# jiaxi98/cnf_ot

Hardware: AMD Instinct MI355X
Metric: MC samples/sec through flow fwd+log|detJ| at dim=2, batch=65536 (higher is better)
Workload: dtype f32; 1 GPU; configs[1]: OT free dim=2, batch=65536, sample_and_log_prob (RQS fwd + log|detJ|), L=2 H=16 M=2 K=5, params N(0,0.20^2) seed 42; ONE STEP = one evaluator-shaped pass of 10000 time-slices x 65536 samples (cnf_ot/utils.py:311-340), each slice its own condition t, one cnf_sample_logprob call per rank; batch=65536, dim=2, parallelism=slice-shard x1 (contiguous blocks of the step's slices; no collective)

## Files before the change

cnf_ot_amd/csrc/cnf_flow.hip:

```cpp
#include "cnf_common.h"
#include <cstdlib>
#include "cnf_pwl_build.h"

#include <math.h>
#include <new>
#include <stdlib.h>
#include <string.h>

namespace cnf {


enum CMode { C_SINGLE = 0, C_PER_SAMPLE = 1, C_TILE_UNIFORM = 2, C_GENERIC = 3 };
enum AuxMode { AUX_LOGDET = 0, AUX_LOGPROB = 1 };


template <class R> struct FlowArgsT {
  ModelArgs m;
  const R* in;
  const R* c;
  R* out;
  R* aux;
  int64_t B;
  int64_t c_block;
  int32_t c_mode, aux_mode;
// ... 296 lines not shown
    T o, ld, olo;
    const bool last = step == a.L - 1;
    [[maybe_unused]] R* clo = nullptr;
    if constexpr (PRECISE) {
      clo = LO + SPL * threadIdx.x;
      const T vlo = step == 0 ? splat<T>(0.0f) : lds_get<T>(clo, first_idx, TS);
      table_spline_precise<K, FAST>(tab, tabd, lds_get<T>(cu, first_idx, TS), vlo, sc, o, ld, olo);
      lds_put(clo, first_idx, TS, olo);
      if (last) bacc->add(o, olo);
    } else {
      table_spline<K, INV, FAST, T>(tab, lds_get<T>(cu, first_idx, TS), sc, o, ld);
    }
    lds_put(co, first_idx, TS, o);
    acc += ld;
    uniform_ptr w = weights + l * a.per_layer;
    const float* wq = a.wq + l * a.per_layer_q;
    for (int d = 1; d < D; ++d) {
      const int i = first_idx + d * idx_step;
      T th[P];
      if constexpr (MFMA && !std::is_same<T, double>::value) {
        conditioner_mfma<T>(reinterpret_cast<const f4*>(wq), d, a.M, c, TO_BASE ? co : cu, first_idx, idx_step, TS, th,
                            D >= 3 ? w : nullptr);
        wq += cond_floats_mfma(d, a.M);
        w += cond_floats(d, H, a.M, P);
      } else {
        conditioner<H, P, T, PERIODIC>(w, d, a.M, c, TO_BASE ? co : cu, first_idx, idx_step, TS, th);
        w += cond_floats_p(d, H, a.M, P, PERIODIC);
      }
      if constexpr (PRECISE) {
        const T vlo = step == 0 ? splat<T>(0.0f) : lds_get<T>(clo, i, TS);
        cond_spline_precise<K, FAST, false>(th, lds_get<T>(cu, i, TS), vlo, sc, a.scd, e2tab, o, ld, olo);
        lds_put(clo, i, TS, olo);
        if (last) bacc->add(o, olo);
      } else {
        cond_spline<K, INV, FAST, T>(th, lds_get<T>(cu, i, TS), sc, o, ld);
      }
      lds_put(co, i, TS, o);
      acc += ld;
    }
    R* t = U; U = O; O = t;
  }
  return acc;
}

__device__ __forceinline__ void store_aux(float* aux, int64_t i, int64_t B, float r) {
  if (i < B) aux[i] = r;
}
__device__ __forceinline__ void store_aux(double* aux, int64_t i, int64_t B, double r) {
  if (i < B) aux[i] = r;
}
__device__ __forceinline__ void store_aux(float* aux, int64_t i, int64_t B, v2f r) {
  if (i + 1 < B && ((reinterpret_cast<uintptr_t>(aux + i) & 7) == 0)) *reinterpret_cast<v2f*>(aux + i) = r;
  else { if (i < B) aux[i] = r.x; if (i + 1 < B) aux[i + 1] = r.y; }
}

template <int H, int K, bool TO_BASE, bool FAST, class T, bool MFMA = false, bool PRECISE = false, bool PERIODIC = false, int DFIX = 0>
__global__ __launch_bounds__(TILE, 2) void flow_kernel(const FlowArgsT<typename Lanes<T>::real> a) {
  typedef typename Lanes<T>::real R;
  extern __shared__ __attribute__((aligned(16))) float lds_raw[];
  R* lds = reinterpret_cast<R*>(lds_raw);
  constexpr int HDR = hdr_floats(K);
  constexpr int SPL = Lanes<T>::N;
  constexpr int TS = TILE * SPL;
  const int DD = DFIX ? DFIX : a.m.D;
  const uint32_t dmagic = DFIX == 2 ? 0x80000000u : (uint32_t)a.div_magic;
  R* tab = lds;
  R* U = lds + HDR;
  R* O = U + DD * TS;
  if (gate_closed(a)) return;
  for (int i = threadIdx.x; i < HDR; i += TILE) tab[i] = table_of<R>(a.m)[i];
  [[maybe_unused]] double* e2tab = nullptr;
  [[maybe_unused]] double* tabd = nullptr;
  [[maybe_unused]] R* LO = nullptr;
  if constexpr (PRECISE) {
    LO = O + DD * TS;
    e2tab = reinterpret_cast<double*>(LO + DD * TS);
    tabd = e2tab + EXP2_N;
    for (int i = threadIdx.x; i < EXP2_N; i += TILE) e2tab[i] = a.m.e2tab[i];
    for (int i = threadIdx.x; i < HDR; i += TILE) tabd[i] = a.m.tabd[i];
  }

  const int64_t n_tiles = (a.B + TS - 1) / TS;
  for (int64_t tile = blockIdx.x; tile < n_tiles; tile += gridDim.x) {
    const int64_t tile_start = tile * TS;
    const int64_t i = tile_start + SPL * threadIdx.x;
    __syncthreads();
    if (TO_BASE && !PRECISE && a.fd2) tile_load_fd<R>(a, U, DD, dmagic, TS, tile_start);
    else if (a.in) tile_load<R>(a.in, U, DD, dmagic, TS, tile_start, a.B);
    else tile_noise_flow(a, U, DD, dmagic, TS, tile_start, TILE);
    const T c = load_cond<T>(a, tile_start, i);
    __syncthreads();

    T base = splat<T>(0.0f);
    if (!TO_BASE && a.aux_mode == AUX_LOGPROB && a.aux) base = base_logprob<T>(lds_col<T>(U + SPL * threadIdx.x, TS), DD);
    BaseAcc<T> bacc;
    [[maybe_unused]] T poison = splat<T>(0.0f);
    if constexpr (TO_BASE) {
      for (int d = 0; d < DD; ++d) { const T v = lds_get<T>(U + SPL * threadIdx.x, d, TS); poison += v - v; }
    }
    const T acc = flow_pass<H, K, TO_BASE, FAST, T, MFMA, PRECISE, PERIODIC, DFIX>(a.m, tab, U, O, c, e2tab, tabd, LO, &bacc);
    if (a.aux) {
      T r = acc;
      if (a.aux_mode == AUX_LOGPROB) {
        if constexpr (PRECISE) r = bacc.log_prob(acc, DD);
        else r = TO_BASE ? base_logprob<T>(lds_col<T>(U + SPL * threadIdx.x, TS), DD) + acc : base - acc;
      }
      if constexpr (TO_BASE) r += poison;
      if (TO_BASE && !PRECISE && a.fd2) store_fd(a, i, r);
      else store_aux(a.aux, i, a.B, r);
    }
    if (a.out) {
      if constexpr (TO_BASE) {
        for (int d = 0; d < DD; ++d) lds_put(U + SPL * threadIdx.x, d, TS, lds_get<T>(U + SPL * threadIdx.x, d, TS) + poison);
      }
      __syncthreads();
      tile_store<R>(a.out, U, DD, dmagic, TS, tile_start, a.B);
    }
  }
}


template <class R>
__device__ __forceinline__ void tile_load_n(const R* __restrict__ g, R* U, int D, uint32_t magic, int TS,
                                            int64_t tile_start, int64_t B, int nthreads) {
  const int64_t base = tile_start * D;
  const int n_el = (int)(B - tile_start < TS ? B - tile_start : TS) * D;
  for (int e = threadIdx.x; e < TS * D; e += nthreads) {
    const int s = magic ? (int)__umulhi((uint32_t)e, magic) : e, d = e - s * D;
    U[d * TS + s] = e < n_el ? g[base + e] : (R)0;
  }
}
template <class R>
__device__ __forceinline__ void tile_store_n(R* __restrict__ g, const R* U, int D, uint32_t magic, int TS,
                                             int64_t tile_start, int64_t B, int nthreads) {
  const int64_t base = tile_start * D;
  const int n_el = (int)(B - tile_start < TS ? B - tile_start : TS) * D;
  for (int e = threadIdx.x; e < n_el; e += nthreads) {
    const int s = magic ? (int)__umulhi((uint32_t)e, magic) : e, d = e - s * D;
    g[base + e] = U[d * TS + s];
  }
}

template <int H, int K, bool FAST, class T>
__global__ __launch_bounds__(1024) void flow_dpar_kernel(const FlowArgs a) {
  extern __shared__ __attribute__((aligned(16))) float lds[];
  constexpr int HDR = hdr_floats(K), P = 3 * K + 1, SPL = Lanes<T>::N, TS = 64 * SPL;
  const int D = a.m.D, L = a.m.L, NT = blockDim.x, NW = NT >> 6;
  const int wave = __builtin_amdgcn_readfirstlane(threadIdx.x >> 6), lane = threadIdx.x & 63;
  float* tab = lds;
  float* U = lds + HDR;
  float* O = U + D * TS;
  float* LD = O + D * TS;
  if (gate_closed(a)) return;
  for (int i = threadIdx.x; i < HDR; i += NT) tab[i] = a.m.prep[i];
  const SplineConsts& sc = a.m.sc;
  uniform_ptr weights = as_uniform(a.m.prep + HDR);
  const int64_t cpart = cond_floats(0, H, a.m.M, P) - H;

  const int64_t n_tiles = (a.B + TS - 1) / TS;
  for (int64_t tile = blockIdx.x; tile < n_tiles; tile += gridDim.x) {
    const int64_t tile_start = tile * TS;
    const int64_t i = tile_start + SPL * lane;
    __syncthreads();
    if (a.in) tile_load_n<float>(a.in, U, D, a.div_magic, TS, tile_start, a.B, NT);
    else tile_noise_flow(a, U, D, a.div_magic, TS, tile_start, NT);
    const T c = load_cond<T>(a, tile_start, i);
    __syncthreads();
    T base = splat<T>(0.0f);
    if (wave == 0 && a.aux_mode == AUX_LOGPROB && a.aux) base = base_logprob<T>(lds_col<T>(U + SPL * lane, TS), D);
    T acc = splat<T>(0.0f);
    for (int l = 0; l < L; ++l) {
      const bool odd = l & 1;
      const int first_idx = odd ? D - 1 : 0, idx_step = odd ? -1 : 1;
      const float* cu = U + SPL * lane;
      float* co = O + SPL * lane;
      T o, ld;
      if (wave == 0) {
        table_spline<K, true, FAST, T>(tab, lds_get<T>(cu, first_idx, TS), sc, o, ld);
        lds_put(co, first_idx, TS, o);
        acc += ld;
      }
      for (int d = 1 + wave; d < D; d += NW) {
        const int64_t off = l * a.m.per_layer + (int64_t)H * ((d - 1) + (int64_t)d * (d - 1) / 2) + (d - 1) * cpart;
        T th[P];
        conditioner<H, P, T>(weights + off, d, a.m.M, c, cu, first_idx, idx_step, TS, th);
        const int idx = first_idx + d * idx_step;
        cond_spline<K, true, FAST, T>(th, lds_get<T>(cu, idx, TS), sc, o, ld);
        lds_put(co, idx, TS, o);
        acc += ld;
      }
      __syncthreads();
      float* t = U; U = O; O = t;
    }
    if (a.aux) lds_put(LD + wave * TS + SPL * lane, 0, TS, acc);
    __syncthreads();
    if (a.aux && wave == 0) {
      T tot = splat<T>(0.0f);
      for (int w = 0; w < NW; ++w) tot += lds_get<T>(LD + w * TS + SPL * lane, 0, TS);
      store_aux(a.aux, i, a.B, a.aux_mode == AUX_LOGPROB ? base - tot : tot);
    }
    if (a.out) tile_store_n<float>(a.out, U, D, a.div_magic, TS, tile_start, a.B, NT);
  }
}

constexpr int PWL_MAX_THREADS = 1024;

struct PwlArgs {
  ModelArgs m;
  const float* in;
  float* out;
  float* aux;
  const float* tables;
  int64_t B, slice_len;
  int32_t n_slices, tiles_per_slice, aux_mode;
  const uint32_t* gate;
  uint32_t gate_epoch;
  int32_t gate_want;
  uint64_t seed;
  int64_t first_sample, slice_stride;
  int32_t in_shared;
};

__global__ void cond_uniform_kernel(const float* __restrict__ c, int64_t B, uint32_t* flag, uint32_t epoch) {
  const uint32_t c0 = __float_as_uint(c[0]);
  bool diff = false;
  for (int64_t i = blockIdx.x * (int64_t)blockDim.x + threadIdx.x; i < B; i += (int64_t)gridDim.x * blockDim.x)
    diff |= __float_as_uint(c[i]) != c0;
  if (__syncthreads_or(diff) && threadIdx.x == 0) *flag = epoch;
}

template <int K, bool TO_BASE, bool FAST, bool PRECISE = false, bool SHIFT_FREE_OK = false, int LROWS = PWL_LROWS, int LFIX = 0,
          bool LEAN_OK = false>
__device__ __forceinline__ v2f flow2_tables(const float* tab, const float* tbl, const float* __restrict__ gtbl,
                                            int L, const SplineConsts sc, v2f& u0, v2f& u1,
                                            const PreciseConsts* pc = nullptr, const double* e2tab = nullptr,
                                            const double* tabd = nullptr, BaseAcc<v2f>* bacc = nullptr) {
  constexpr bool INV = !TO_BASE;
  constexpr bool LEAN = LEAN_OK && INV && FAST;
  static_assert(!PRECISE || TO_BASE, "precise path: data -> base");
  v2f acc = splat<v2f>(0.0f);
  [[maybe_unused]] v2f lo0 = splat<v2f>(0.0f), lo1 = lo0;
  if (LFIX) L = LFIX;
#pragma unroll
  for (int step = 0; step < (LFIX ? LFIX : L); ++step) {
    const int l = TO_BASE ? L - 1 - step : step;
    const bool odd = l & 1;
    const v2f uf = odd ? u1 : u0, uo = odd ? u0 : u1;
    v2f of, oo, ld, olo_f, olo_o;
    bool general;
    const float* tl = tbl + l * pwl_ltbl(LROWS);
    const float* gl = gtbl + (int64_t)l * PWL_TBL;
    if constexpr (PRECISE) {
      table_spline_precise<K, FAST>(tab, tabd, uf, odd ? lo1 : lo0, sc, of, ld, olo_f);
      if (step == L - 1) bacc->add(of, olo_f);
      acc += ld;
      v2f th[PWL_P];
      pwl_eval<LROWS>(tl, gl, of, th, general);
      cond_spline_precise<K, FAST, true>(th, uo, odd ? lo0 : lo1, sc, *pc, e2tab, oo, ld, olo_o);
      if (step == L - 1) bacc->add(oo, olo_o);
      lo0 = odd ? olo_o : olo_f;
      lo1 = odd ? olo_f : olo_o;
    } else {
      PwlRows rr;
      v2f qa[K], qb[K];
      if (!TO_BASE) {
        pwl_find<LROWS>(tl, uf, rr, general);
        rr.dua = pwl_logit_pairs<LROWS>(rr.ra, gl, rr.pa, uf.x, qa);
        rr.dub = pwl_logit_pairs<LROWS>(rr.rb, gl, rr.pb, uf.y, qb);
      }
      constexpr bool LOGPROD = LEAN;
      bool tails = true;
      if constexpr (LEAN) tails = __builtin_amdgcn_ballot_w64(maybe_outside(uf, uo, sc.lo, sc.hi)) != 0;
      v2f larg = splat<v2f>(1.0f);
      if constexpr (LOGPROD) {
        table_spline<K, INV, FAST, v2f, true, LEAN>(tab, uf, sc, of, larg, tails);
      } else {
        table_spline<K, INV, FAST, v2f, false, LEAN>(tab, uf, sc, of, ld, tails);
        acc += ld;
      }
      if (TO_BASE) {
        pwl_find<LROWS>(tl, of, rr, general);
        rr.dua = pwl_logit_pairs<LROWS>(rr.ra, gl, rr.pa, of.x, qa);
        rr.dub = pwl_logit_pairs<LROWS>(rr.rb, gl, rr.pb, of.y, qb);
      }
      auto slopes = [&](int ka, int kb, v2f& ta, v2f& tb) {
        ta = pwl_slope_pair<LROWS>(rr.ra, gl, rr.pa, ka, rr.dua);
        tb = pwl_slope_pair<LROWS>(rr.rb, gl, rr.pb, kb, rr.dub);
      };
      if (!SHIFT_FREE_OK || __builtin_amdgcn_ballot_w64(general) != 0)
      {
        cond_spline_rows<K, INV, FAST, false, false, LEAN>(qa, qb, slopes, uo, sc, oo, ld, tails);
        if constexpr (LOGPROD) { const v2f lg = Math<FAST>::log(larg); ld += INV ? -lg : lg; }
      } else {
        cond_spline_rows<K, INV, FAST, true, LOGPROD, LEAN>(qa, qb, slopes, uo, sc, oo, ld, tails);
        if constexpr (LOGPROD) { const v2f lg = Math<FAST>::log(larg * ld); ld = INV ? -lg : lg; }
      }
    }
    acc += ld;
    u0 = odd ? oo : of;
    u1 = odd ? of : oo;
  }
  return acc;
}

template <int K, bool TO_BASE, bool FAST, bool PRECISE = false, int LROWS = PWL_LROWS, int LFIX = 0, bool SEEDED = false>
__global__ __launch_bounds__(PWL_MAX_THREADS) void flow_pwl_kernel(const PwlArgs a) {
  const int PWL_THREADS = blockDim.x, PWL_TS = 2 * PWL_THREADS;
  extern __shared__ __attribute__((aligned(16))) float lds_raw[];
  constexpr int HDR = (hdr_floats(K) + 3) & ~3;
  float* tab = lds_raw;
  float* tbl = lds_raw + HDR;
  const int tid = threadIdx.x;
  const int L = LFIX ? LFIX : a.m.L;
  if (gate_closed(a)) return;
  for (int i = tid; i < hdr_floats(K); i += PWL_THREADS) tab[i] = table_of<float>(a.m)[i];
  const SplineConsts sc = sc_scalars(sc_of<float>(a.m));
  [[maybe_unused]] double* e2tab = nullptr;
  [[maybe_unused]] double* tabd = nullptr;
  if constexpr (PRECISE) {
    e2tab = reinterpret_cast<double*>(tbl + L * pwl_ltbl(LROWS));
    tabd = e2tab + EXP2_N;
    for (int i = tid; i < EXP2_N; i += PWL_THREADS) e2tab[i] = a.m.e2tab[i];
    for (int i = tid; i < hdr_floats(K); i += PWL_THREADS) tabd[i] = a.m.tabd[i];
  }

  const int total = a.n_slices * a.tiles_per_slice;
  const int per_block = (total + gridDim.x - 1) / gridDim.x;
  const int t0 = blockIdx.x * per_block;
  const int t1 = t0 + per_block < total ? t0 + per_block : total;
  int cur = -1;
  struct Tile { int slice; int ti; int valid; int64_t g0; int64_t st0; int64_t gin; };
  auto tile_at = [&](int slice, int ti) {
    Tile t;
    t.slice = slice;
    t.ti = ti;
    const int64_t s0 = (int64_t)t.slice * a.slice_len;
    const int64_t len = a.B - s0 < a.slice_len ? a.B - s0 : a.slice_len;
    const int64_t jt = (int64_t)ti * PWL_TS;
    const int64_t left = len - jt;
    t.valid = left >= PWL_TS ? PWL_TS : (left > 0 ? (int)left : 0);
    t.g0 = s0 + jt;
    t.gin = a.in_shared ? jt : t.g0;
    t.st0 = a.first_sample + (int64_t)t.slice * a.slice_stride + jt;
    return t;
  };
  auto tile_of = [&](int tile) { const int sl = tile / a.tiles_per_slice; return tile_at(sl, tile - sl * a.tiles_per_slice); };
  auto tile_next = [&](const Tile& t) {
    return t.ti + 1 < a.tiles_per_slice ? tile_at(t.slice, t.ti + 1) : tile_at(t.slice + 1, 0);
  };
  const uint32_t lane2 = 2u * (uint32_t)tid;
  auto tile_points = [&](const Tile& t) {
    f4 x = {0.f, 0.f, 0.f, 0.f};
    if (SEEDED && !a.in) {
      const uint64_t e0 = (uint64_t)(t.st0 + lane2) * 2u;
      if ((int)lane2 < t.valid) {
        if ((e0 & 3) == 0) {
          float z[4];
          philox_normals4(a.seed, e0 >> 2, z);
#pragma unroll
          for (int q = 0; q < 4; ++q) x[q] = z[q];
        } else {
#pragma unroll
          for (int q = 0; q < 4; ++q) x[q] = normal_at(a.seed, e0 + q);
        }
        if ((int)lane2 + 1 >= t.valid) { x[2] = 0.f; x[3] = 0.f; }
      }
      return x;
    }
    const float* p = a.in + 2 * t.gin;
    if (t.valid == PWL_TS) x = *reinterpret_cast<const f4*>(p + 2u * lane2);
    else if ((int)lane2 + 1 < t.valid) x = *reinterpret_cast<const f4*>(p + 2u * lane2);
    else if ((int)lane2 < t.valid) { x[0] = p[2u * lane2]; x[1] = p[2u * lane2 + 1]; }
    return x;
  };
  [[maybe_unused]] f4 xn = {0.f, 0.f, 0.f, 0.f};
  Tile tn{};
  if (t0 < t1) { tn = tile_of(t0); xn = tile_points(tn); }
  for (int tile = t0; tile < t1; ++tile) {
    const Tile tl = tn;
    const int slice = tl.slice;
    if (slice != cur) {
      __syncthreads();
      pwl_stage<LROWS>(tbl, a.tables + (int64_t)slice * L * PWL_TBL, L, tid, PWL_THREADS);
      cur = slice;
      __syncthreads();
    }
    const bool full = tl.valid == PWL_TS;
    const bool v0 = (int)lane2 < tl.valid, v1 = (int)lane2 + 1 < tl.valid;
    const f4 x = xn;
    if (tile + 1 < t1) { tn = tile_next(tl); xn = tile_points(tn); }
    __builtin_amdgcn_sched_barrier(0);
    v2f u0 = {x[0], x[2]}, u1 = {x[1], x[3]};
    [[maybe_unused]] v2f poison = splat<v2f>(0.0f);
    if constexpr (TO_BASE) poison = (u0 - u0) + (u1 - u1);

    v2f base = splat<v2f>(0.0f);
    if (!TO_BASE && a.aux_mode == AUX_LOGPROB && a.aux) base = (u0 * u0 + u1 * u1) * -0.5f - (float)(2 * HALF_LOG_2PI);
    BaseAcc<v2f> bacc;
    const v2f acc = flow2_tables<K, TO_BASE, FAST, PRECISE, true, LROWS, LFIX, true>(tab, tbl, a.tables + (int64_t)slice * L * PWL_TBL, L, sc,
                                                            u0, u1, &a.m.scd, e2tab, tabd, &bacc);
    if (a.aux) {
      v2f r = acc;
      if constexpr (PRECISE) { if (a.aux_mode == AUX_LOGPROB) r = bacc.log_prob(acc, 2); }
      else if (a.aux_mode == AUX_LOGPROB)
        r = TO_BASE ? (u0 * u0 + u1 * u1) * -0.5f - (float)(2 * HALF_LOG_2PI) + acc : base - acc;
      if constexpr (TO_BASE) r += poison;
      float* q = a.aux + tl.g0;
      if (full || v1) *reinterpret_cast<v2f*>(q + lane2) = r;
      else if (v0) q[lane2] = r.x;
    }
    if (a.out) {
      float* q = a.out + 2 * tl.g0;
      if constexpr (TO_BASE) { u0 += poison; u1 += poison; }
      if (full || v1) *reinterpret_cast<f4*>(q + 2u * lane2) = f4{u0.x, u1.x, u0.y, u1.y};
      else if (v0) { q[2u * lane2] = u0.x; q[2u * lane2 + 1] = u1.x; }
    }
  }
}

struct LossArgs {
  ModelArgs m;
  CnfLossSpec spec;
  const float* pts;
  const float* t;
  double* sums;
  int64_t B;
  int64_t n_slices;
  int64_t pts_slice_stride;
  uint32_t div_magic;
  uint64_t seed;
  int64_t first_sample;
  DensityMix mix;
};

template <class T>
__device__ __forceinline__ void copy_cols(float* dst, const float* src, int D, int TS) {
  for (int d = 0; d < D; ++d) lds_put(dst, d, TS, lds_get<T>(src, d, TS));
}

__device__ __forceinline__ float mask_tail(float v, int64_t i, int64_t B) { return i < B ? v : 0.0f; }
__device__ __forceinline__ float mask_tail(v2f v, int64_t i, int64_t B) {
  return (i < B ? v.x : 0.0f) + (i + 1 < B ? v.y : 0.0f);
}

template <int H, int K, bool FAST, class T>
__global__ __launch_bounds__(TILE, 2) void loss_kernel(const LossArgs a) {
  extern __shared__ __attribute__((aligned(16))) float lds[];
  constexpr int HDR = hdr_floats(K);
  constexpr int SPL = Lanes<T>::N;
  constexpr int TS = TILE * SPL;
  using M = Math<FAST>;
  const int D = a.m.D;
  float* tab = lds;
  float* Nn = lds + HDR;
  float* U = Nn + D * TS;
  float* O = U + D * TS;
  float* V = O + D * TS;
  float* R = V + D * TS;
  for (int i = threadIdx.x; i < HDR; i += TILE) tab[i] = a.m.prep[i];
  const int col = SPL * threadIdx.x;
  const int kind = a.spec.kind;

  const int64_t tiles_per_slice = (a.B + TS - 1) / TS;
  const int64_t n_tiles = tiles_per_slice * a.n_slices;
  SliceSum ssum;
  for (int64_t tile = blockIdx.x; tile < n_tiles; tile += gridDim.x) {
    const int64_t slice = tile / tiles_per_slice;
    const int64_t tile_start = (tile - slice * tiles_per_slice) * TS;
    const int64_t i = tile_start + col;
    __syncthreads();
    if (a.pts)
      tile_load<float>(a.pts + slice * a.pts_slice_stride * D, Nn, D, a.div_magic, TS, tile_start, a.B);
    else
      tile_noise(a.seed, (uint64_t)(a.first_sample + slice * a.pts_slice_stride + tile_start) * (uint64_t)D, Nn, D,
                 a.div_magic, TS, a.B - tile_start);
    const float t = a.t[slice];
    __syncthreads();

    T acc = splat<T>(0.0f);
    const float dt = a.spec.dt;
    const bool kin = kind <= CNF_TERM_FLOW_MATCHING;
    const bool data = kind == CNF_TERM_NEG_LOGPROB || kind == CNF_TERM_DENSITY_L2_DATA;
    const int n_fwd = data ? 0 : (kind == CNF_TERM_KINETIC ? 2 : (kin ? 3 : 1));
    T fldj = splat<T>(0.0f);
    for (int p = 0; p < n_fwd; ++p) {
      const float c = !kin ? t : (p == 0 ? t - 0.5f * dt : (p == 1 ? t + 0.5f * dt : t));
      copy_cols<T>(U + col, Nn + col, D, TS);
      fldj = flow_pass<H, K, false, FAST, T>(a.m, tab, U, O, splat<T>(c));
      if (kin) {
        if (p == 0) copy_cols<T>(V + col, U + col, D, TS);
        else if (p == 1) {
          const float inv_dt = 1.0f / dt;
          for (int d = 0; d < D; ++d)
            lds_put(V + col, d, TS, (lds_get<T>(U + col, d, TS) - lds_get<T>(V + col, d, TS)) * inv_dt);
        } else copy_cols<T>(R + col, U + col, D, TS);
      }
    }
    if (kind == CNF_TERM_KINETIC) {
      acc = sq_norm<T>(lds_col<T>(V + col, TS), D);
    } else if (kind == CNF_TERM_POTENTIAL) {
      acc = potential<FAST, T>(lds_col<T>(U + col, TS), D, a.spec.subtype, a.spec.a).v;
    } else if (kind == CNF_TERM_REVERSE_KL) {
      const T lp = base_logprob<T>(lds_col<T>(Nn + col, TS), D) - fldj;
      acc = lp - rkl_mixture<FAST, T>(lds_col<T>(U + col, TS), D, t, a.spec.T, a.spec.beta).logmix;
    } else if (kind == CNF_TERM_DENSITY_L2) {
      const T lp = base_logprob<T>(lds_col<T>(Nn + col, TS), D) - fldj;
      acc = density_l2_residual<FAST, T>(lp, density_mixture<FAST, T>(lds_col<T>(U + col, TS), D, t, a.mix));
    }
    const bool neg = data;
    const int n_tb = neg ? 1 : ((kind == CNF_TERM_KINETIC_SCORE || kind == CNF_TERM_FLOW_MATCHING) ? 2 * D : 0);
    const float dx = a.spec.dx;
    T lp0 = splat<T>(0.0f);
    for (int e = 0; e < n_tb; ++e) {
      const int d = e >> 1, sgn = e & 1;
      copy_cols<T>(U + col, (neg ? Nn : R) + col, D, TS);
      if (!neg) lds_put(U + col, d, TS, lds_get<T>(R + col, d, TS) + (sgn == 0 ? 0.5f * dx : -0.5f * dx));
      if (kind == CNF_TERM_DENSITY_L2_DATA)
        lds_put(V + col, 0, TS, density_mixture<FAST, T>(lds_col<T>(Nn + col, TS), D, t, a.mix));
      const T ildj = flow_pass<H, K, true, FAST, T>(a.m, tab, U, O, splat<T>(t));
      const T lp = base_logprob<T>(lds_col<T>(U + col, TS), D) + ildj;
      if (kind == CNF_TERM_DENSITY_L2_DATA) acc = density_l2_residual<FAST, T>(lp, lds_get<T>(V + col, 0, TS));
      else if (neg) acc = -lp;
      else if (sgn == 0) lp0 = lp;
      else {
        const T dr = drift_field<T>(lds_col<T>(R + col, TS), d, kind == CNF_TERM_FLOW_MATCHING ? a.spec.subtype : -1, a.spec.a);
        const T u = score_residual(lds_get<T>(V + col, d, TS), (lp0 - lp) * (1.0f / dx), a.spec.coef, dr);
        acc = vfma(u, u, acc);
      }
    }
    float part = mask_tail(acc, i, a.B);
#pragma unroll
    for (int off = 32; off > 0; off >>= 1) part += __shfl_xor(part, off, 64);
    ssum.add(a.sums, slice, part);
  }
  ssum.flush(a.sums);
}


template <class R> struct FieldArgsT {
  ModelArgs m;
  const R* pts;
  const R* t;
  const R* fixed;
  const R* sec;
  R* rho;
  R* logp;
  R* vel;
  R* score;
  R* traj;
  double lo_x, lo_y, step_x, step_y;
  int64_t N, S;
  int32_t nx, axis_x, axis_y, sec_axis, n_sec;
  int32_t fixed_base;
  int32_t slice_chunk;
  R t0, dt, dx;
  uint32_t div_magic;
};

template <class T>
__device__ __forceinline__ void field_copy(typename Lanes<T>::real* dst, const typename Lanes<T>::real* src, int D) {
  for (int d = 0; d < D; ++d) lds_put(dst, d, TILE, lds_get<T>(src, d, TILE));
}
template <class T>
__device__ __forceinline__ T field_poison(const typename Lanes<T>::real* col, int D) {
  T p = (T)0;
  for (int d = 0; d < D; ++d) { const T v = lds_get<T>(col, d, TILE); p += v - v; }
  return p;
}

template <int H, int K, bool FAST, class T>
__global__ __launch_bounds__(TILE, 2) void fields_kernel(const FieldArgsT<T> a) {
  static_assert(Lanes<T>::N == 1, "one point per lane");
  typedef T R;
  constexpr bool PR = std::is_same<T, float>::value;
  extern __shared__ __attribute__((aligned(16))) float lds_raw[];
  R* lds = reinterpret_cast<R*>(lds_raw);
  constexpr int HDR = hdr_floats(K);
  constexpr int TS = TILE;
  const int D = a.m.D;
  R* tab = lds;
  R* P = lds + HDR;
  R* U = P + D * TS;
  R* O = U + D * TS;
  R* X = O + D * TS;
  R* V = X + D * TS;
  for (int i = threadIdx.x; i < HDR; i += TILE) tab[i] = table_of<R>(a.m)[i];
  [[maybe_unused]] double* e2tab = nullptr;
  [[maybe_unused]] double* tabd = nullptr;
  [[maybe_unused]] R* LO = nullptr;
  if constexpr (PR) {
    LO = V + D * TS;
    e2tab = reinterpret_cast<double*>(LO + D * TS);
    tabd = e2tab + EXP2_N;
    for (int i = threadIdx.x; i < EXP2_N; i += TILE) e2tab[i] = a.m.e2tab[i];
    for (int i = threadIdx.x; i < HDR; i += TILE) tabd[i] = a.m.tabd[i];
  }
  const int col = threadIdx.x;
  const bool want_xi = a.vel || a.traj;
  const bool want_base = want_xi || a.rho || a.logp;
  const R half_dt = (R)0.5 * a.dt, inv_dt = (R)1 / a.dt, half_dx = (R)0.5 * a.dx, inv_dx = (R)1 / a.dx;

  const int64_t tiles = (a.N + TS - 1) / TS;
  const int64_t chunks = (a.S + a.slice_chunk - 1) / a.slice_chunk;
  for (int64_t item = blockIdx.x; item < tiles * chunks; item += gridDim.x) {
    const int64_t chunk = item / tiles;
    const int64_t tile_start = (item - chunk * tiles) * TS;
    const int64_t i = tile_start + col;
    const int64_t s0 = chunk * a.slice_chunk, s1 = s0 + a.slice_chunk < a.S ? s0 + a.slice_chunk : a.S;
    __syncthreads();
    if (a.pts) {
      tile_load<R>(a.pts, P, D, a.div_magic, TS, tile_start, a.N);
    } else {
      const int64_t n = i < a.N ? i : 0;
      const int64_t iy = n / a.nx, ix = n - iy * a.nx;
      for (int d = 0; d < D; ++d) lds_put(P + col, d, TS, a.fixed[d]);
      if (a.sec) lds_put(P + col, a.sec_axis, TS, a.sec[0]);
      lds_put(P + col, a.axis_x, TS, (R)__dadd_rn(__dmul_rn((double)ix, a.step_x), a.lo_x));
      lds_put(P + col, a.axis_y, TS, (R)__dadd_rn(__dmul_rn((double)iy, a.step_y), a.lo_y));
    }
    __syncthreads();

    T poison = (T)0;
    for (int64_t s = s0; s < s1; ++s) {
      const R ts = a.t[s];
      if (want_base && (s == s0 || !a.fixed_base)) {
        double rho_acc = 0.0;
        T lp = (T)0;
        for (int k = 0; k < a.n_sec; ++k) {
          field_copy<T>(U + col, P + col, D);
          if (a.sec) lds_put(U + col, a.sec_axis, TS, a.sec[k]);
          poison = field_poison<T>(U + col, D);
          BaseAcc<T> bacc;
          const T ildj = flow_pass<H, K, true, FAST, T, false, PR>(a.m, tab, U, O, a.fixed_base ? a.t0 : ts, e2tab, tabd,
                                                                   LO, &bacc);
          if constexpr (PR) lp = bacc.log_prob(ildj, D) + poison;
          else lp = base_logprob<T>(lds_col<T>(U + col, TS), D) + ildj + poison;
          rho_acc += exp((double)lp);
        }
        if (want_xi) field_copy<T>(X + col, U + col, D);
        if (a.logp && i < a.N) a.logp[s * a.N + i] = lp;
        if (a.rho && i < a.N) a.rho[s * a.N + i] = (R)(rho_acc / (double)a.n_sec);
      }
      const int n_fwd = (a.traj ? 1 : 0) + (a.vel ? 2 : 0);
      for (int p = 0; p < n_fwd; ++p) {
        const int q = p - (a.traj ? 1 : 0);
        const R c = q < 0 ? ts : (q == 0 ? ts - half_dt : ts + half_dt);
        field_copy<T>(U + col, X + col, D);
        (void)flow_pass<H, K, false, FAST, T>(a.m, tab, U, O, c);
        if (q == 0) { field_copy<T>(V + col, U + col, D); continue; }
        for (int d = 0; d < D; ++d) {
          const T r = lds_get<T>(U + col, d, TS);
          lds_put(V + col, d, TS, q < 0 ? r + poison : (r - lds_get<T>(V + col, d, TS)) * inv_dt + poison);
        }
        __syncthreads();
        tile_store<R>((q < 0 ? a.traj : a.vel) + s * a.N * D, V, D, a.div_magic, TS, tile_start, a.N);
        __syncthreads();
      }
      if (a.score) {
        T lp0 = (T)0;
        for (int e = 0; e < 2 * D; ++e) {
          const int d = e >> 1, sgn = e & 1;
          field_copy<T>(U + col, P + col, D);
          lds_put(U + col, d, TS, lds_get<T>(P + col, d, TS) + (sgn == 0 ? half_dx : -half_dx));
          const T ps = field_poison<T>(U + col, D);
          const T ildj = flow_pass<H, K, true, FAST, T>(a.m, tab, U, O, ts);
          const T lp = base_logprob<T>(lds_col<T>(U + col, TS), D) + ildj;
          if (sgn == 0) lp0 = lp;
          else lds_put(V + col, d, TS, (lp0 - lp) * inv_dx + ps);
        }
        __syncthreads();
        tile_store<R>(a.score + s * a.N * D, V, D, a.div_magic, TS, tile_start, a.N);
        __syncthreads();
      }
    }
  }
}


struct LossPwlArgs {
  ModelArgs m;
  CnfLossSpec spec;
  const float* pts;
  const float* t;
  double* sums;
  const float* tables;
  int64_t B, n_slices, pts_slice_stride;
  uint64_t seed;
  int64_t first_sample;
  int32_t n_sets, tiles_per_slice;
  DensityMix mix;
};

template <int K, bool FAST>
__global__ __launch_bounds__(PWL_MAX_THREADS) void loss_pwl_kernel(const LossPwlArgs a) {
  using M = Math<FAST>;
  typedef v2f T;
  const int NT = blockDim.x, TS = 2 * NT;
  extern __shared__ __attribute__((aligned(16))) float lds_raw[];
  constexpr int HDR = (hdr_floats(K) + 3) & ~3;
  const int tid = threadIdx.x;
  const int L = a.m.L;
  float* tab = lds_raw;
  float* tbl = lds_raw + HDR;
  float* R = tbl + a.n_sets * L * PWL_LTBL;
  for (int i = tid; i < hdr_floats(K); i += NT) tab[i] = table_of<float>(a.m)[i];
  const SplineConsts sc = sc_scalars(sc_of<float>(a.m));
  const int kind = a.spec.kind;
  const bool kin = kind <= CNF_TERM_FLOW_MATCHING;
  const float dt = a.spec.dt, dx = a.spec.dx;
  const int64_t set_stride = a.n_slices * L * (int64_t)PWL_TBL;
  const int col = 2 * tid;

  const int total = (int)a.n_slices * a.tiles_per_slice;
  const int per_block = (total + gridDim.x - 1) / gridDim.x;
  const int t0 = blockIdx.x * per_block;
  const int t1 = t0 + per_block < total ? t0 + per_block : total;
  int cur = -1;
  SliceSum ssum;
  for (int tile = t0; tile < t1; ++tile) {
    const int slice = tile / a.tiles_per_slice;
    __syncthreads();
// ... 1084 lines not shown
```

cnf_ot_amd/csrc/cnf_pwl.h:

```cpp
#pragma once

#include "cnf_common.h"

namespace cnf {

constexpr int PWL_H = 16;
constexpr int PWL_P = 16;
constexpr int PWL_NBP = 320;
constexpr int PWL_NG = 2048;
constexpr int PWL_NPIECE = 289;
constexpr float PWL_GMIN = -16.0f;
constexpr float PWL_GSCALE = 64.0f;
constexpr uint32_t PWL_G_INDEX = 0x1ff, PWL_G_MANY = 0x4000, PWL_G_GENERAL = 0x8000;
constexpr int PWL_NREF = 304;
constexpr int PWL_OFF_GRID = PWL_NBP;
constexpr int PWL_OFF_REF = PWL_NBP + PWL_NG / 2;
constexpr int PWL_OFF_PIECE = PWL_NBP + PWL_NG / 2 + PWL_NREF;
static_assert(PWL_OFF_PIECE % 4 == 0, "rows are read with 16-byte LDS loads");
constexpr int PWL_ROW = 36;
constexpr int PWL_TBL = PWL_OFF_PIECE + PWL_NPIECE * PWL_ROW;
constexpr int PWL_LROWS = 112;
constexpr int PWL_LTBL = PWL_OFF_PIECE + PWL_LROWS * PWL_ROW;
constexpr int pwl_ltbl(int lrows) { return PWL_OFF_PIECE + lrows * PWL_ROW; }
constexpr int PWL_N_SLOT = PWL_NBP - 1;


constexpr double PWL_FAST_LOGIT = 4.0;
constexpr double PWL_FAST_SLOPE_LO = -3.0;
constexpr double PWL_FAST_SLOPE_HI = 40.0;
constexpr int PWL_CHUNK = 64;


__device__ __forceinline__ float fma_scalar(float a, float b, float c) {
  float r;
  asm("v_fma_f32 %0, %1, %2, %3" : "=v"(r) : "v"(a), "v"(b), "v"(c));
  return r;
}

typedef const f4 __attribute__((address_space(3))) * lds_f4_ptr;

__device__ __forceinline__ int pwl_cell(float u) {
  const int cell = (int)fmaf(u, PWL_GSCALE, -PWL_GMIN * PWL_GSCALE);
  return cell < 0 ? 0 : (cell > PWL_NG - 1 ? PWL_NG - 1 : cell);
}

template <int LROWS = PWL_LROWS>
__device__ __forceinline__ void pwl_row(const float* tbl, const float* __restrict__ gtbl, int p, float u,
                                        float (&th)[PWL_P]) {
  const float du = u - tbl[PWL_OFF_REF + p];
  if (LROWS >= PWL_NPIECE || p < LROWS) {
    const lds_f4_ptr row = (lds_f4_ptr)(uintptr_t)((uint32_t)(uintptr_t)(tbl + PWL_OFF_PIECE) + __umul24((uint32_t)p, PWL_ROW * 4));
#pragma unroll
    for (int q = 0; q < 4; ++q) {
      const f4 s = row[q], t = row[4 + q];
#pragma unroll
      for (int e = 0; e < 4; ++e) th[4 * q + e] = fma_scalar(s[e], du, t[e]);
    }
  } else {
    const f4* row = reinterpret_cast<const f4*>(gtbl + PWL_OFF_PIECE + p * PWL_ROW);
#pragma unroll
    for (int q = 0; q < 4; ++q) {
      const f4 s = row[q], t = row[4 + q];
#pragma unroll
      for (int e = 0; e < 4; ++e) th[4 * q + e] = fma_scalar(s[e], du, t[e]);
    }
  }
}

__device__ __forceinline__ int pwl_piece(const float* tbl, float u, bool& general) {
  const uint32_t g = reinterpret_cast<const uint16_t*>(tbl + PWL_OFF_GRID)[pwl_cell(u)];
  general = (g & PWL_G_GENERAL) != 0;
  int p = (int)(g & PWL_G_INDEX);
  const float us = u;
  const float b0 = tbl[p], b1 = tbl[p + 1];
  p += (b0 <= us ? 1 : 0) + (b1 <= us ? 1 : 0);
  if (g & PWL_G_MANY) while (tbl[p] <= us) ++p;
  return p;
}
__device__ __forceinline__ void pwl_piece(const float* tbl, v2f u, int& px, int& py, bool& general) {
  const uint16_t* grid = reinterpret_cast<const uint16_t*>(tbl + PWL_OFF_GRID);
  const uint32_t gx = grid[pwl_cell(u.x)], gy = grid[pwl_cell(u.y)];
  general = ((gx | gy) & PWL_G_GENERAL) != 0;
  px = (int)(gx & PWL_G_INDEX); py = (int)(gy & PWL_G_INDEX);
  const float ux = u.x, uy = u.y;
  const float ax0 = tbl[px], ax1 = tbl[px + 1], ay0 = tbl[py], ay1 = tbl[py + 1];
  px += (ax0 <= ux ? 1 : 0) + (ax1 <= ux ? 1 : 0);
  py += (ay0 <= uy ? 1 : 0) + (ay1 <= uy ? 1 : 0);
  if ((gx | gy) & PWL_G_MANY) {
    bool more;
    do {
      const bool mx = tbl[px] <= ux, my = tbl[py] <= uy;
      px += mx ? 1 : 0;
      py += my ? 1 : 0;
      more = mx || my;
    } while (more);
  }
}

template <int LROWS = PWL_LROWS>
__device__ __forceinline__ void pwl_eval(const float* tbl, const float* __restrict__ gtbl, float u, float (&th)[PWL_P],
                                         bool& general) {
  const int p = pwl_piece(tbl, u, general);
  pwl_row<LROWS>(tbl, gtbl, p, u, th);
}

template <int LROWS = PWL_LROWS>
__device__ __forceinline__ void pwl_eval(const float* tbl, const float* __restrict__ gtbl, v2f u, v2f (&th)[PWL_P],
                                         bool& general) {
  int px, py;
  pwl_piece(tbl, u, px, py, general);
  float tx[PWL_P], ty[PWL_P];
  pwl_row<LROWS>(tbl, gtbl, px, u.x, tx);
  pwl_row<LROWS>(tbl, gtbl, py, u.y, ty);
#pragma unroll
  for (int m = 0; m < PWL_P; ++m) th[m] = v2f{tx[m], ty[m]};
}

typedef const float __attribute__((address_space(3))) * lds_f_ptr;
typedef const v2f __attribute__((address_space(3))) * lds_v2_ptr;

struct PwlRows {
  int pa, pb;
  float dua, dub;
  lds_f_ptr ra, rb;
};

template <int LROWS>
__device__ __forceinline__ lds_f_ptr pwl_lds_row(const float* tbl, int p) {
  const uint32_t q = LROWS >= PWL_NPIECE ? (uint32_t)p : (uint32_t)(p < LROWS ? p : LROWS - 1);
  static_assert(PWL_ROW == 36, "row stride 144 B = 9 << 4");
  uint32_t q9 = (q << 3) + q;
  asm volatile("" : "+v"(q9));
  return (lds_f_ptr)(uintptr_t)((uint32_t)(uintptr_t)(tbl + PWL_OFF_PIECE) + (q9 << 4));
}

template <int LROWS>
__device__ __forceinline__ void pwl_find(const float* tbl, v2f u, PwlRows& r, bool& general) {
  int px, py;
  pwl_piece(tbl, u, px, py, general);
  r.pa = px; r.pb = py;
  r.ra = pwl_lds_row<LROWS>(tbl, px);
  r.rb = pwl_lds_row<LROWS>(tbl, py);
}

template <class FP, class F4P, class V2P>
__device__ __forceinline__ float pwl_logit_pairs_(FP r, F4P r4, V2P r2, float u, v2f (&q)[5]) {
  const f4 s0 = r4[0], s1 = r4[1], t0 = r4[4], t1 = r4[5];
  const v2f s2 = r2[4], t2 = r2[12];
  const float du = u - r[2 * PWL_P];
  const v2f d2 = v2f{du, du};
  q[0] = __builtin_elementwise_fma(__builtin_shufflevector(s0, s0, 0, 1), d2, __builtin_shufflevector(t0, t0, 0, 1));
  q[1] = __builtin_elementwise_fma(__builtin_shufflevector(s0, s0, 2, 3), d2, __builtin_shufflevector(t0, t0, 2, 3));
  q[2] = __builtin_elementwise_fma(__builtin_shufflevector(s1, s1, 0, 1), d2, __builtin_shufflevector(t1, t1, 0, 1));
  q[3] = __builtin_elementwise_fma(__builtin_shufflevector(s1, s1, 2, 3), d2, __builtin_shufflevector(t1, t1, 2, 3));
  q[4] = __builtin_elementwise_fma(s2, d2, t2);
  return du;
}

template <int LROWS>
__device__ __forceinline__ float pwl_logit_pairs(lds_f_ptr row, const float* __restrict__ gtbl, int p, float u,
                                                 v2f (&q)[5]) {
  float du = pwl_logit_pairs_(row, (lds_f4_ptr)row, (lds_v2_ptr)row, u, q);
  if (LROWS < PWL_NPIECE && p >= LROWS) {
    const float* g = gtbl + PWL_OFF_PIECE + p * PWL_ROW;
    du = pwl_logit_pairs_(g, reinterpret_cast<const f4*>(g), reinterpret_cast<const v2f*>(g), u, q);
  }
  return du;
}

template <int LROWS>
__device__ __forceinline__ v2f pwl_slope_pair(lds_f_ptr row, const float* __restrict__ gtbl, int p, int k, float du) {
  const v2f d2 = v2f{du, du};
  const lds_f_ptr r = row + k;
  v2f t = __builtin_elementwise_fma(v2f{r[10], r[11]}, d2, v2f{r[PWL_P + 10], r[PWL_P + 11]});
  if (LROWS < PWL_NPIECE && p >= LROWS) {
    const float* g = gtbl + PWL_OFF_PIECE + p * PWL_ROW + k;
    t = __builtin_elementwise_fma(v2f{g[10], g[11]}, d2, v2f{g[PWL_P + 10], g[PWL_P + 11]});
  }
  return t;
}

template <int LROWS, int NT>
__device__ __forceinline__ float pwl_row_dot(lds_f_ptr row, const float* __restrict__ gtbl, int p, int k,
                                             const float (&t)[NT], float s0, float s1) {
  static_assert(NT == 10, "K = 5");
  auto dot = [&](f4 a, f4 b, v2f c, float k0, float k1) {
    float r = k0 * s0;
    r = fmaf(k1, s1, r);
#pragma unroll
    for (int e = 0; e < 4; ++e) { r = fmaf(a[e], t[e], r); r = fmaf(b[e], t[4 + e], r); }
    r = fmaf(c.x, t[8], r);
    return fmaf(c.y, t[9], r) * 0.693147182464599609375f;
  };
  const lds_f_ptr rk = row + k;
  float r = dot(((lds_f4_ptr)row)[0], ((lds_f4_ptr)row)[1], ((lds_v2_ptr)row)[4], rk[10], rk[11]);
  if (LROWS < PWL_NPIECE && p >= LROWS) {
    const float* g = gtbl + PWL_OFF_PIECE + p * PWL_ROW;
    r = dot(reinterpret_cast<const f4*>(g)[0], reinterpret_cast<const f4*>(g)[1], reinterpret_cast<const v2f*>(g)[4], g[10 + k], g[11 + k]);
  }
  return r;
}

template <int LROWS = PWL_LROWS>
__device__ __forceinline__ void pwl_stage(float* tbl, const float* __restrict__ g0, int L, int tid, int nthreads) {
  for (int l = 0; l < L; ++l) {
    const float* g = g0 + (int64_t)l * PWL_TBL;
    const int n = __float_as_int(g[PWL_N_SLOT]);
    const int rows = n + 1 < LROWS ? n + 1 : LROWS;
    const f4* src = reinterpret_cast<const f4*>(g);
    f4* dst = reinterpret_cast<f4*>(tbl + l * pwl_ltbl(LROWS));
    for (int i = tid; i < (PWL_OFF_PIECE + rows * PWL_ROW) / 4; i += nthreads) dst[i] = src[i];
  }
}

}
```

Baseline: 89.59 billion samples/s.

## Prefetch next slice's spline tables into registers before the slice handover

When the next tile belongs to a new time slice, each thread loads its share of that slice's piece tables from global memory into registers one tile early. At the handover these registers are written to LDS instead of doing a cold global-to-LDS copy, and the size header for the slice after that is also read ahead. The aim is to hide global-load latency at the barrier-bracketed slice switch. In exchange the kernel holds more live registers, which may lower occupancy, and it gains optional clock64 timing stamps behind a debug macro.

```diff
diff --git a/cnf_ot_amd/csrc/cnf_flow.hip b/cnf_ot_amd/csrc/cnf_flow.hip
--- a/cnf_ot_amd/csrc/cnf_flow.hip
+++ b/cnf_ot_amd/csrc/cnf_flow.hip
@@ -622,6 +622,14 @@
   }
   return acc;
 }
+
+#ifdef CNF_HANDOVER_STAMPS
+constexpr int PWL_STAMP_BLOCKS = 1024;
+__device__ unsigned long long pwl_stamp_buf[4 * PWL_STAMP_BLOCKS];
+#define PWL_STAMP(x) x
+#else
+#define PWL_STAMP(x)
+#endif
 
 template <int K, bool TO_BASE, bool FAST, bool PRECISE = false, int LROWS = PWL_LROWS, int LFIX = 0, bool SEEDED = false>
 __global__ __launch_bounds__(PWL_MAX_THREADS) void flow_pwl_kernel(const PwlArgs a) {
@@ -696,19 +704,35 @@
   [[maybe_unused]] f4 xn = {0.f, 0.f, 0.f, 0.f};
   Tile tn{};
   if (t0 < t1) { tn = tile_of(t0); xn = tile_points(tn); }
+  auto tables_of = [&](int slice) { return a.tables + (int64_t)slice * L * PWL_TBL; };
+  constexpr int AHEAD_NL = SEEDED || PRECISE || LROWS < PWL_NPIECE ? 1 : (LFIX ? LFIX : 2);
+  constexpr bool AHEAD = !(SEEDED && LROWS < PWL_NPIECE);
+  PwlAhead<LROWS, AHEAD_NL, 1> ahead;
+  PWL_STAMP(unsigned long long st_hand = 0; unsigned long long st_first = 0; unsigned long long st_n = 0;)
+  PWL_STAMP(const unsigned long long st_loop = clock64();)
   for (int tile = t0; tile < t1; ++tile) {
     const Tile tl = tn;
     const int slice = tl.slice;
     if (slice != cur) {
+      PWL_STAMP(const unsigned long long st_in = clock64();)
       __syncthreads();
-      pwl_stage<LROWS>(tbl, a.tables + (int64_t)slice * L * PWL_TBL, L, tid, PWL_THREADS);
+      if (AHEAD && ahead.slice == slice) ahead.put(tbl, tables_of(slice), L, tid, PWL_THREADS);
+      else pwl_stage<LROWS>(tbl, tables_of(slice), L, tid, PWL_THREADS);
+      __syncthreads();
+      PWL_STAMP(const unsigned long long st_d = clock64() - st_in; st_hand += st_d; st_n += 1; if (cur < 0) st_first = st_d;)
       cur = slice;
-      __syncthreads();
     }
     const bool full = tl.valid == PWL_TS;
     const bool v0 = (int)lane2 < tl.valid, v1 = (int)lane2 + 1 < tl.valid;
     const f4 x = xn;
-    if (tile + 1 < t1) { tn = tile_next(tl); xn = tile_points(tn); }
+    if (tile + 1 < t1) {
+      tn = tile_next(tl); xn = tile_points(tn);
+      if (AHEAD && tn.slice != slice) ahead.get(tables_of(tn.slice), L, tn.slice, tid, PWL_THREADS);
+      if (AHEAD && tile + 2 < t1) {
+        const int s2 = tn.ti + 1 < a.tiles_per_slice ? tn.slice : tn.slice + 1;
+        if (s2 != slice && s2 != ahead.cnt_slice) ahead.sizes(tables_of(s2), L, s2);
+      }
+    }
     __builtin_amdgcn_sched_barrier(0);
     v2f u0 = {x[0], x[2]}, u1 = {x[1], x[3]};
     [[maybe_unused]] v2f poison = splat<v2f>(0.0f);
@@ -717,7 +741,7 @@
     v2f base = splat<v2f>(0.0f);
     if (!TO_BASE && a.aux_mode == AUX_LOGPROB && a.aux) base = (u0 * u0 + u1 * u1) * -0.5f - (float)(2 * HALF_LOG_2PI);
     BaseAcc<v2f> bacc;
-    const v2f acc = flow2_tables<K, TO_BASE, FAST, PRECISE, true, LROWS, LFIX, true>(tab, tbl, a.tables + (int64_t)slice * L * PWL_TBL, L, sc,
+    const v2f acc = flow2_tables<K, TO_BASE, FAST, PRECISE, true, LROWS, LFIX, true>(tab, tbl, tables_of(slice), L, sc,
                                                             u0, u1, &a.m.scd, e2tab, tabd, &bacc);
     if (a.aux) {
       v2f r = acc;
@@ -736,7 +760,30 @@
       else if (v0) { q[2u * lane2] = u0.x; q[2u * lane2 + 1] = u1.x; }
     }
   }
-}
+#ifdef CNF_HANDOVER_STAMPS
+  if (tid == 0 && blockIdx.x < PWL_STAMP_BLOCKS) {
+    unsigned long long* s = pwl_stamp_buf + 4 * blockIdx.x;
+    s[0] += st_hand; s[1] += clock64() - st_loop; s[2] += st_n; s[3] += st_first;
+  }
+#endif
+}
+
+#ifdef CNF_HANDOVER_STAMPS
+}
+extern "C" int cnf_debug_handover_stamps(unsigned long long* out, int n, int reset) {
+  if (n < 0 || n > cnf::PWL_STAMP_BLOCKS) return CNF_ERR_INVALID;
+  const size_t bytes = sizeof(unsigned long long) * 4 * (size_t)n;
+  if (hipDeviceSynchronize() != hipSuccess) return CNF_ERR_HIP;
+  if (out && hipMemcpyFromSymbol(out, HIP_SYMBOL(cnf::pwl_stamp_buf), bytes) != hipSuccess) return CNF_ERR_HIP;
+  if (reset) {
+    void* p = nullptr;
+    if (hipGetSymbolAddress(&p, HIP_SYMBOL(cnf::pwl_stamp_buf)) != hipSuccess) return CNF_ERR_HIP;
+    if (hipMemset(p, 0, sizeof(cnf::pwl_stamp_buf)) != hipSuccess) return CNF_ERR_HIP;
+  }
+  return CNF_OK;
+}
+namespace cnf {
+#endif
 
 struct LossArgs {
   ModelArgs m;
diff --git a/cnf_ot_amd/csrc/cnf_pwl.h b/cnf_ot_amd/csrc/cnf_pwl.h
--- a/cnf_ot_amd/csrc/cnf_pwl.h
+++ b/cnf_ot_amd/csrc/cnf_pwl.h
@@ -202,15 +202,65 @@
 }
 
 template <int LROWS = PWL_LROWS>
-__device__ __forceinline__ void pwl_stage(float* tbl, const float* __restrict__ g0, int L, int tid, int nthreads) {
-  for (int l = 0; l < L; ++l) {
+__device__ __forceinline__ int pwl_stage_f4s(const float* __restrict__ g) {
+  const int n = __float_as_int(g[PWL_N_SLOT]);
+  const int rows = n + 1 < LROWS ? n + 1 : LROWS;
+  return (PWL_OFF_PIECE + rows * PWL_ROW) / 4;
+}
+
+template <int LROWS = PWL_LROWS>
+__device__ __forceinline__ void pwl_stage(float* tbl, const float* __restrict__ g0, int L, int tid, int nthreads,
+                                          int l0 = 0) {
+  for (int l = l0; l < L; ++l) {
     const float* g = g0 + (int64_t)l * PWL_TBL;
-    const int n = __float_as_int(g[PWL_N_SLOT]);
-    const int rows = n + 1 < LROWS ? n + 1 : LROWS;
+    const int cnt = pwl_stage_f4s<LROWS>(g);
     const f4* src = reinterpret_cast<const f4*>(g);
     f4* dst = reinterpret_cast<f4*>(tbl + l * pwl_ltbl(LROWS));
-    for (int i = tid; i < (PWL_OFF_PIECE + rows * PWL_ROW) / 4; i += nthreads) dst[i] = src[i];
-  }
-}
-
-}
+    for (int i = tid; i < cnt; i += nthreads) dst[i] = src[i];
+  }
+}
+
+template <int LROWS, int NL, int Q>
+struct PwlAhead {
+  int cnt_slice = -1;
+  int slice = -1;
+  int cnt[NL], vcnt[NL];
+  f4 v[NL][Q];
+
+  __device__ __forceinline__ void sizes(const float* __restrict__ g0, int L, int s) {
+#pragma unroll
+    for (int l = 0; l < NL; ++l)
+      if (l < L) cnt[l] = __builtin_amdgcn_readfirstlane(pwl_stage_f4s<LROWS>(g0 + (int64_t)l * PWL_TBL));
+    cnt_slice = s;
+  }
+  __device__ __forceinline__ void get(const float* __restrict__ g0, int L, int s, int tid, int nthreads) {
+    if (cnt_slice != s) sizes(g0, L, s);
+#pragma unroll
+    for (int l = 0; l < NL; ++l) {
+      if (l < L) {
+        vcnt[l] = cnt[l];
+        const f4* src = reinterpret_cast<const f4*>(g0 + (int64_t)l * PWL_TBL);
+#pragma unroll
+        for (int q = 0; q < Q; ++q)
+          if (tid + q * nthreads < vcnt[l]) v[l][q] = src[tid + q * nthreads];
+      }
+    }
+    slice = s;
+  }
+  __device__ __forceinline__ void put(float* tbl, const float* __restrict__ g0, int L, int tid, int nthreads) const {
+#pragma unroll
+    for (int l = 0; l < NL; ++l) {
+      if (l < L) {
+        const f4* src = reinterpret_cast<const f4*>(g0 + (int64_t)l * PWL_TBL);
+        f4* dst = reinterpret_cast<f4*>(tbl + l * pwl_ltbl(LROWS));
+#pragma unroll
+        for (int q = 0; q < Q; ++q)
+          if (tid + q * nthreads < vcnt[l]) dst[tid + q * nthreads] = v[l][q];
+        for (int i = tid + Q * nthreads; i < vcnt[l]; i += nthreads) dst[i] = src[i];
+      }
+    }
+    pwl_stage<LROWS>(tbl, g0, L, tid, nthreads, NL);
+  }
+};
+
+}
```

Result: slower. 87.67 billion samples/s (-2.1%).
